# bcsefercik/markerless-robot-camera-calibration

Hardware: AMD Instinct MI355X
Metric: point-cloud frames/sec at 200k pts/frame (higher is better)
Workload: dtype f32

## Files before the change

### markerless-robot-camera-calibration_amd/csrc/sv_conv.hip

```cpp
#include <stdio.h>
#include <stdlib.h>
#include <array>
#include <utility>
#include <vector>

#include "sv_conv_params.h"

namespace sv {

static thread_local char g_last_instance[128] = "";
static thread_local double g_want_scale_override = -1.0;
static thread_local double g_tail_override = -1.0;

constexpr int lds_row_stride(int kc) {
  for (int sa = kc + 2;; ++sa)
    if (sa % 64 == 34 || (sa % 4 == 0 && (sa / 4) % 2 == 1)) return sa;
}

template <int TM_, int WAVES_N, int NT, int CPO = 0>
struct ConvCfg {
  static constexpr ConvTile T = conv_tile(TM_, WAVES_N, NT, CPO);
  static constexpr int WAVES_M = 4 / WAVES_N;
  static constexpr int MR = T.mr, TN = T.tn, GK = T.gk, KC = T.kc, PFD = T.pfd;
  static constexpr bool USE_FULL = T.use_full;
  static constexpr int SA = lds_row_stride(KC);
  static constexpr int F4_PER_ROW = KC / 4;
  static constexpr int ROWS_PER_PASS = 256 / F4_PER_ROW;
  static constexpr int A_F4 = (TM_ + ROWS_PER_PASS - 1) / ROWS_PER_PASS;
  static_assert(MR >= 1, "tile too small for the wave layout");
  static constexpr size_t lds_bytes(int K) { return (size_t)(2 * TM_ * SA + K * TM_) * sizeof(float); }
};

template <int TM_, int WAVES_N, int NT, bool FAST, int CPO = 0, bool RING = false, bool FULL = false>
__device__ __forceinline__ void conv_tile_body(const ConvParams& p, const int bidx, const int tile_base) {
  static_assert(FAST || !FULL, "FULL is a refinement of the FAST form");
  using Cfg = ConvCfg<TM_, WAVES_N, NT, CPO>;
  constexpr int MR = Cfg::MR, TN = Cfg::TN, A_F4 = Cfg::A_F4, KC = Cfg::KC, SA = Cfg::SA, GK = Cfg::GK;
  constexpr int PFD = RING ? Cfg::PFD : 1;
  constexpr int ROWS_PER_PASS = Cfg::ROWS_PER_PASS;
  constexpr int SUBS = TM_ / 16;
  constexpr bool WIDE = FAST && !FULL && !RING && CPO == 0 && WAVES_N == 4 && NT == 3 && (TM_ == 64 || TM_ == 32);
  static_assert(!WIDE || A_F4 == 2, "the WIDE step moves a step's gathers in two halves");
  extern __shared__ __attribute__((aligned(16))) float lds[];
  float* As = lds;
  int* idx_s = (int*)(lds + 2 * TM_ * SA);

  const int tid = threadIdx.x;
  const int lane = tid & 63;
  const int wid = __builtin_amdgcn_readfirstlane(tid >> 6);
  const int wm = wid / WAVES_N, wn = wid % WAVES_N;
  unsigned long long trace_t0 = 0, trace_t_loop = 0, trace_t_epi = 0;
  int trace_steps = 0;
  if (p.trace) trace_t0 = wall_clock64();
  const int ny = (p.Cout + TN - 1) / TN;
  constexpr int SUB_PER_PLAN_TILE = PLAN_TILE / TM_;
  const int t_lin = bidx / ny;
  const int t128 = tile_base + t_lin / SUB_PER_PLAN_TILE;
  const int p128 = p.tile_order ? p.tile_order[t128] : ((int)(p.Vpad / PLAN_TILE) - 1 - t128);
  const int tile = p128 * SUB_PER_PLAN_TILE + (t_lin % SUB_PER_PLAN_TILE);
  const int n0 = (bidx % ny) * TN;
  const int64_t row0 = (int64_t)tile * TM_;
  const int li = lane & 15, lq = lane >> 4;
  const int K = p.K, Cin = p.Cin, Cout = p.Cout;
  const int col0 = n0 + wn * NT * 16 + NT * li;
  const bool cols_full = col0 + NT <= Cout;

  f32x4 acc[MR][NT];
#pragma unroll
  for (int s = 0; s < MR; ++s)
#pragma unroll
    for (int n = 0; n < NT; ++n) acc[s][n] = (f32x4){0.f, 0.f, 0.f, 0.f};

  if (p.acc_init) {
    if constexpr (FAST) {
      const __amdgpu_buffer_rsrc_t rsrc_acc = __builtin_amdgcn_make_buffer_rsrc((void*)p.acc_init, 0, (int)p.acc_bytes, 0x00020000);
      int o_acc[MR][4];
      load_perm_rows<MR>(p, row0 + wm * MR * 16, lane >> 4, o_acc);
#pragma unroll
      for (int s = 0; s < MR; ++s)
#pragma unroll
        for (int reg = 0; reg < 4; ++reg) {
          const auto v = buffer_load_floats<NT>(
              rsrc_acc, o_acc[s][reg] >= 0 ? (uint32_t)o_acc[s][reg] * (uint32_t)(p.acc_ld * 4) + (uint32_t)col0 * 4u : BUF_ABSENT, 0u);
#pragma unroll
          for (int n = 0; n < NT; ++n) acc[s][n][reg] = v[n];
        }
    } else {
#pragma unroll
      for (int s = 0; s < MR; ++s)
#pragma unroll
        for (int reg = 0; reg < 4; ++reg) {
          const int64_t r = row0 + wm * MR * 16 + s * 16 + (lane >> 4) * 4 + reg;
          const int64_t o = p.perm ? (int64_t)p.perm[r] : (r < p.V_out ? r : -1);
#pragma unroll
          for (int n = 0; n < NT; ++n) acc[s][n][reg] = (o >= 0 && col0 + n < Cout) ? p.acc_init[o * p.acc_ld + col0 + n] : 0.0f;
        }
    }
  }
  uint32_t dense_mask = (1u << SUBS) - 1u;
  if (p.submask == nullptr) {
    const int64_t rem = p.V_out - row0;
    const int nsub = rem >= TM_ ? SUBS : (int)((rem + 15) / 16);
    dense_mask = (1u << nsub) - 1u;
  }
  if constexpr (FAST) {
    constexpr int STAGE_IT = (32 * TM_ + 255) / 256;
    int n_st[STAGE_IT];
#pragma unroll
    for (int it = 0; it < STAGE_IT; ++it) {
      const int e = tid + 256 * it;
      const int k = e / TM_, r = e % TM_;
      n_st[it] = -1;
      if (e < K * TM_) {
        if (p.nbr_s)
          n_st[it] = p.nbr_s[(int64_t)k * p.Vpad + row0 + r];
        else
          n_st[it] = (row0 + r < p.V_out) ? (int)(row0 + r) : -1;
      }
    }
#pragma unroll
    for (int it = 0; it < STAGE_IT; ++it) {
      const int e = tid + 256 * it;
      if (e < K * TM_) idx_s[e] = (int)(n_st[it] >= 0 ? (uint32_t)n_st[it] * (uint32_t)(p.in_ld * 4) : BUF_ABSENT);
    }
  } else {
    for (int e = tid; e < K * TM_; e += 256) {
      const int k = e / TM_, r = e - k * TM_;
      int n;
      if (p.nbr_s)
        n = p.nbr_s[(int64_t)k * p.Vpad + row0 + r];
      else
        n = (row0 + r < p.V_out) ? (int)(row0 + r) : -1;
      idx_s[e] = n;
    }
  }
  const __amdgpu_buffer_rsrc_t rsrc_in = __builtin_amdgcn_make_buffer_rsrc((void*)p.in, 0, (int)p.in_bytes, 0x00020000);
  const __amdgpu_buffer_rsrc_t rsrc_w = __builtin_amdgcn_make_buffer_rsrc((void*)p.W, 0, (int)p.w_bytes, 0x00020000);

  const int64_t sm_word = row0 / PLAN_TILE;
  const int sm_shift = (int)((row0 % PLAN_TILE) / 16);
  uint32_t my_sm = 0;
  if (lane < K) my_sm = p.submask ? ((p.submask[sm_word * K + lane] >> sm_shift) & ((1u << SUBS) - 1u)) : dense_mask;
  const uint32_t amask = (uint32_t)__ballot(my_sm != 0);
  auto fused_mask = [&](int k0) -> uint32_t {
    uint32_t m = 0;
#pragma unroll
    for (int g = 0; g < GK; ++g) m |= (uint32_t)__builtin_amdgcn_readlane((int)my_sm, min(k0 + g, 31));
    return m;
  };
  int k_n, c_n = 0;
  uint32_t sm_n = 0;
  bool have_n;
  if (CPO) {
    k_n = 0;
    while (k_n < K && (sm_n = fused_mask(k_n)) == 0) k_n += GK;
    have_n = k_n < K;
  } else {
    k_n = amask ? __builtin_ctz(amask) : K;
    sm_n = amask ? (uint32_t)__builtin_amdgcn_readlane((int)my_sm, k_n) : 0u;
    have_n = amask != 0;
  }
  auto advance = [&]() {
    if (CPO) {
      k_n += GK;
      while (k_n < K && (sm_n = fused_mask(k_n)) == 0) k_n += GK;
      have_n = k_n < K;
      return;
    }
    c_n += KC;
    if (c_n >= Cin) {
      c_n = 0;
      const uint32_t rest = amask & ~((2u << k_n) - 1u);
      have_n = rest != 0;
      k_n = have_n ? __builtin_ctz(rest) : K;
      sm_n = (uint32_t)__builtin_amdgcn_readlane((int)my_sm, have_n ? k_n : 0);
    }
  };

  float4 ra[A_F4];
  const int a_cc = (tid % Cfg::F4_PER_ROW) * 4;
  const int a_r = tid / Cfg::F4_PER_ROW;

  const uint32_t col_bytes = (uint32_t)a_cc * 4u;
  const int cin_rem = Cin % KC;
  const uint32_t col_last = (cin_rem == 0 || a_cc < cin_rem) ? col_bytes : 0u - (uint32_t)(Cin - cin_rem) * 4u;
  auto gather_row = [&](int k, int c0, uint32_t sm, int j) -> float4 {
    const int r = a_r + ROWS_PER_PASS * j;
    if (FAST) {
      const int rr = (A_F4 * ROWS_PER_PASS > TM_) ? min(r, TM_ - 1) : r;
      if (CPO) {
        const int kk = k + a_cc / (CPO ? CPO : 1);
        uint32_t off = (uint32_t)idx_s[min(kk, K - 1) * TM_ + rr];
        if (kk >= K) off = BUF_ABSENT;
        const f32x4 v = buffer_load_floats<4>(rsrc_in, off + (uint32_t)(a_cc % (CPO ? CPO : 1)) * 4u, 0u);
        return make_float4(v[0], v[1], v[2], v[3]);
      } else {
        const uint32_t off = (uint32_t)idx_s[k * TM_ + rr];
        const uint32_t cb = (!FULL && c0 + KC > Cin) ? col_last : col_bytes;
        const f32x4 v = buffer_load_floats<4>(rsrc_in, off + cb, (uint32_t)c0 * 4u);
        return make_float4(v[0], v[1], v[2], v[3]);
      }
      (void)sm;
    } else if (CPO) {
      float e[4] = {0.f, 0.f, 0.f, 0.f};
      if (r < TM_ && ((sm >> (r >> 4)) & 1u)) {
#pragma unroll
        for (int q = 0; q < 4; ++q) {
          const int i = a_cc + q, kk = k + i / (CPO ? CPO : 1), c = i % (CPO ? CPO : 1);
          if (i < GK * CPO && kk < K) {
            const int n = idx_s[kk * TM_ + r];
            if (n >= 0) e[q] = p.in[(int64_t)n * p.in_ld + c];
          }
        }
      }
      return make_float4(e[0], e[1], e[2], e[3]);
    } else {
      float4 v = make_float4(0.f, 0.f, 0.f, 0.f);
      if (r < TM_ && ((sm >> (r >> 4)) & 1u)) {
        const int n = idx_s[k * TM_ + r];
        const int c = c0 + a_cc;
        if (n >= 0) {
          const float* src = p.in + (int64_t)n * p.in_ld + c;
          if (p.vec_a) {
            if (c < Cin) v = *(const float4*)src;
          } else {
            if (c + 0 < Cin) v.x = src[0];
            if (c + 1 < Cin) v.y = src[1];
            if (c + 2 < Cin) v.z = src[2];
            if (c + 3 < Cin) v.w = src[3];
          }
        }
      }
      return v;
    }
  };
  auto load_a = [&](int k, int c0, uint32_t sm) {
#pragma unroll
    for (int j = 0; j < A_F4; ++j) ra[j] = gather_row(k, c0, sm, j);
  };
  auto scatter_row = [&](float* dstbuf, uint32_t sm, int j, const float4& v) {
    const int r = a_r + ROWS_PER_PASS * j;
    if (r < TM_ && (FAST || ((sm >> (r >> 4)) & 1u))) {
      float2* dst = (float2*)(dstbuf + r * SA + a_cc);
      dst[0] = make_float2(v.x, v.y);
      dst[1] = make_float2(v.z, v.w);
    }
  };
  auto store_a = [&](float* dstbuf, uint32_t sm) {
#pragma unroll
    for (int j = 0; j < A_F4; ++j) scatter_row(dstbuf, sm, j, ra[j]);
  };

  typedef float bvec_t __attribute__((ext_vector_type(NT)));
  typedef float bvec_load_t __attribute__((ext_vector_type(NT), aligned(4)));
  constexpr int KS = KC / 4;
  constexpr int BR = WIDE ? 4 : KS;
  bvec_t b[BR];
  const int b_off = lq * Cout + col0;
  const uint32_t b_off_bytes = (uint32_t)b_off * 4u;
  auto step_weights = [&](int k, int c0) -> const float* { return p.W + ((int64_t)k * Cin + c0) * Cout; };
  auto cols_of = [&](int k, int c0) { return CPO ? min(GK, K - k) * CPO : min(KC, Cin - c0); };
  auto ksteps_of = [&](int k, int c0) { return (cols_of(k, c0) + 3) >> 2; };
  auto load_b = [&](const float* wstep, int k, int c0, int ksteps_valid, int ks, bvec_t& dst) {
    if (FAST) {
      const uint32_t row = (uint32_t)(k * Cin + c0 + (ks < ksteps_valid ? 4 * ks : 0));
      dst = buffer_load_floats<NT>(rsrc_w, b_off_bytes, row * (uint32_t)Cout * 4u);
      (void)wstep;
    } else {
      const int i = 4 * ks + lq;
      const float* src = p.W + ((int64_t)k * Cin + c0 + i) * Cout + col0;
      const bool row_ok = i < cols_of(k, c0);
#pragma unroll
      for (int n = 0; n < NT; ++n) dst[n] = (row_ok && col0 + n < Cout) ? src[n] : 0.0f;
    }
  };

  __syncthreads();
  if (have_n) {
    int k_c = k_n, c_c = c_n;
    uint32_t sm_c = sm_n;
    load_a(k_c, c_c, sm_c);
#pragma unroll
    for (int ks = 0; ks < BR; ++ks) load_b(step_weights(k_c, c_c), k_c, c_c, ksteps_of(k_c, c_c), ks, b[ks]);
    store_a(As, sm_c);
    advance();
    int k_x = k_n, c_x = c_n;
    uint32_t sm_x = sm_n;
    bool have_x = have_n;
    __syncthreads();
    int buf = 0;
    if (p.trace) trace_t_loop = wall_clock64();

    auto step = [&]() -> bool {
      if (FAST || have_x) load_a(have_x ? k_x : 0, have_x ? c_x : 0, have_x ? sm_x : 0u);
      const float* a_base = As + buf * (TM_ * SA) + (wm * MR * 16 + li) * SA + lq;
      const uint32_t smw = (sm_c >> (wm * MR)) & ((1u << MR) - 1u);
      const int ksteps = ksteps_of(k_c, c_c);
      const int kb = have_x ? k_x : 0;
      const int cb = have_x ? c_x : 0;
      const float* wnext = step_weights(kb, cb);
      const int ksteps_next = ksteps_of(kb, cb);
      {
        auto reload_b = [&](int ks) {
          if (FULL) {
            b[ks] = buffer_load_floats<NT>(rsrc_w, b_off_bytes, (uint32_t)(kb * Cin + cb + 4 * ks) * (uint32_t)Cout * 4u);
          } else if (FAST || have_x) {
            load_b(wnext, kb, cb, ksteps_next, ks, b[ks]);
          }
        };
        auto mfma_row = [&](int ks, const float (&a)[MR]) {
#pragma unroll
          for (int s = 0; s < MR; ++s) {
            if ((MR == 1 && Cfg::WAVES_M == 1) || ((smw >> s) & 1u)) {
#pragma unroll
              for (int n = 0; n < NT; ++n)
                acc[s][n] = __builtin_amdgcn_mfma_f32_16x16x4f32(a[s], b[ks][n], acc[s][n], 0, 0, 0);
            }
          }
        };
        if constexpr (PFD == 1) {
          float a_cur[MR];
#pragma unroll
          for (int s = 0; s < MR; ++s) a_cur[s] = a_base[s * 16 * SA];
#pragma unroll
          for (int ks = 0; ks < KC / 4; ++ks) {
            if (FULL || ks < ksteps) {
              float a_nx[MR];
              if (ks + 1 < KC / 4) {
#pragma unroll
                for (int s = 0; s < MR; ++s) a_nx[s] = a_base[s * 16 * SA + (ks + 1) * 4];
                if (FULL) __builtin_amdgcn_sched_barrier(0);
              }
              mfma_row(ks, a_cur);
              if (ks + 1 < KC / 4) {
#pragma unroll
                for (int s = 0; s < MR; ++s) a_cur[s] = a_nx[s];
              }
            }
            reload_b(ks);
            if (FULL) __builtin_amdgcn_sched_barrier(0);
          }
        } else {
          float a_ring[PFD + 1][MR];
#pragma unroll
          for (int d = 0; d < PFD; ++d)
#pragma unroll
            for (int s = 0; s < MR; ++s) a_ring[d][s] = a_base[s * 16 * SA + d * 4];
#pragma unroll
          for (int ks = 0; ks < KC / 4; ++ks) {
            if (FULL || ks < ksteps) {
              if (ks + PFD < KC / 4) {
#pragma unroll
                for (int s = 0; s < MR; ++s)
                  a_ring[(ks + PFD) % (PFD + 1)][s] = a_base[s * 16 * SA + (ks + PFD) * 4];
                if (FULL) __builtin_amdgcn_sched_barrier(0);
              }
              mfma_row(ks, a_ring[ks % (PFD + 1)]);
            }
            reload_b(ks);
            if (FULL) __builtin_amdgcn_sched_barrier(0);
          }
        }
      }
      ++trace_steps;
      if (!have_x) return false;
      store_a(As + (buf ^ 1) * (TM_ * SA), sm_x);
      k_c = k_x;
      c_c = c_x;
      sm_c = sm_x;
      advance();
      k_x = k_n;
      c_x = c_n;
      sm_x = sm_n;
      have_x = have_n;
      __syncthreads();
      buf ^= 1;
      return true;
    };
    auto step_wide = [&]() -> bool {
      const int kb = have_x ? k_x : 0;
      const int cb = have_x ? c_x : 0;
      float* const a_next = As + (buf ^ 1) * (TM_ * SA);
      ra[0] = gather_row(kb, cb, 0u, 0);
      const float* a_base = As + buf * (TM_ * SA) + (wm * MR * 16 + li) * SA + lq;
      const uint32_t smw = (sm_c >> (wm * MR)) & ((1u << MR) - 1u);
      const int ksteps = ksteps_of(k_c, c_c);
      const int ksteps_next = ksteps_of(kb, cb);
      const uint32_t wrow_c = (uint32_t)(k_c * Cin + c_c);
      const uint32_t wrow_x = (uint32_t)(kb * Cin + cb);
      float a_cur[MR];
#pragma unroll
      for (int s = 0; s < MR; ++s) a_cur[s] = a_base[s * 16 * SA];
#pragma unroll
      for (int ks = 0; ks < KS; ++ks) {
        if (ks < ksteps) {
          float a_nx[MR];
          if (ks + 1 < KS) {
#pragma unroll
            for (int s = 0; s < MR; ++s) a_nx[s] = a_base[s * 16 * SA + (ks + 1) * 4];
          }
#pragma unroll
          for (int s = 0; s < MR; ++s) {
            if ((smw >> s) & 1u) {
#pragma unroll
              for (int n = 0; n < NT; ++n)
                acc[s][n] = __builtin_amdgcn_mfma_f32_16x16x4f32(a_cur[s], b[ks % BR][n], acc[s][n], 0, 0, 0);
            }
          }
          if (ks + 1 < KS) {
#pragma unroll
            for (int s = 0; s < MR; ++s) a_cur[s] = a_nx[s];
          }
        }
        const int kn = ks + BR < KS ? ks + BR : ks + BR - KS;
        const uint32_t wrow = ks + BR < KS ? wrow_c + (uint32_t)(kn < ksteps ? 4 * kn : 0)
                                           : wrow_x + (uint32_t)(kn < ksteps_next ? 4 * kn : 0);
        b[ks % BR] = buffer_load_floats<NT>(rsrc_w, b_off_bytes, wrow * (uint32_t)Cout * 4u);
        if (ks == KS / 2 - 1) {
          scatter_row(a_next, 0u, 0, ra[0]);
          ra[0] = gather_row(kb, cb, 0u, 1);
        }
      }
      ++trace_steps;
      if (!have_x) return false;
      scatter_row(a_next, 0u, 1, ra[0]);
      k_c = k_x;
      c_c = c_x;
      sm_c = sm_x;
      advance();
      k_x = k_n;
      c_x = c_n;
      sm_x = sm_n;
      have_x = have_n;
      __syncthreads();
      buf ^= 1;
      return true;
    };
    if constexpr (WIDE) {
      while (step_wide()) {
      }
    } else {
      while (step()) {
      }
    }
  }

  if (p.trace) trace_t_epi = wall_clock64();
  float sc[NT], sh[NT];
#pragma unroll
  for (int n = 0; n < NT; ++n) {
    const bool ok = col0 + n < Cout;
    sc[n] = (p.scale && ok) ? p.scale[col0 + n] : 1.0f;
    sh[n] = (p.shift && ok) ? p.shift[col0 + n] : 0.0f;
  }
  if constexpr (FAST) {
    epilogue_buffered<MR, NT>(p, acc, row0 + wm * MR * 16, lq, col0);
  } else
#pragma unroll
  for (int s = 0; s < MR; ++s) {
#pragma unroll
    for (int reg = 0; reg < 4; ++reg) {
      const int64_t r = row0 + wm * MR * 16 + s * 16 + lq * 4 + reg;
      int64_t o;
      if (p.perm)
        o = p.perm[r];
      else
        o = (r < p.V_out) ? r : -1;
      if (o < 0) continue;
      float y[NT];
#pragma unroll
      for (int n = 0; n < NT; ++n) {
        float v = acc[s][n][reg];
        if (p.scale)
          v = __builtin_fmaf(v, sc[n], sh[n]);
        else if (p.shift)
          v = v + sh[n];
        y[n] = v;
      }
      if (p.residual) {
        const float* res = p.residual + o * p.res_ld + col0;
#pragma unroll
        for (int n = 0; n < NT; ++n)
          if (col0 + n < Cout) y[n] = y[n] + res[n];
      }
      float* dst = p.out + o * p.out_ld + col0;
#pragma unroll
      for (int n = 0; n < NT; ++n) {
        float v = y[n];
        if (p.act == SV_ACT_RELU)
          v = v < 0.f ? 0.f : v;
        else if (p.act == SV_ACT_LEAKY_RELU)
          v = v > 0.f ? v : v * p.slope;
        if (col0 + n < Cout) dst[n] = v;
      }
    }
  }
  if (p.trace && tid == 0) {
    unsigned long long* t = p.trace + (size_t)blockIdx.x * 4;
    t[0] = trace_t0;
    t[1] = wall_clock64();
    t[2] = ((unsigned long long)__builtin_amdgcn_s_getreg((31 << 11) | 20) << 32) |
           (unsigned)__builtin_amdgcn_s_getreg((31 << 11) | 4);
    const unsigned long long pro = trace_t_loop ? ((trace_t_loop - trace_t0) >> 4) & 0xffffull : 0ull;
    const unsigned long long epi = ((t[1] - trace_t_epi) >> 4) & 0xffffull;
    t[3] = (unsigned long long)(unsigned)trace_steps | (pro << 32) | (epi << 48);
  }
}

constexpr unsigned wide_waves(int tm, int waves_n, int nt, bool fast, int cpo, bool ring, bool full) {
  return (tm == 64 && waves_n == 4 && nt == 3 && fast && cpo == 0 && !ring && !full) ? 5u : 1u;
}

template <int TM_, int WAVES_N, int NT, bool FAST, int CPO = 0, bool RING = false, bool FULL = false>
__global__ __launch_bounds__(256) __attribute__((amdgpu_waves_per_eu(wide_waves(TM_, WAVES_N, NT, FAST, CPO, RING, FULL))))
void conv_fwd_kernel(ConvParams p) {
  conv_tile_body<TM_, WAVES_N, NT, FAST, CPO, RING, FULL>(p, (int)blockIdx.x, 0);
}

template <int TM_, int TAIL_TM, int WAVES_N, int NT, bool FAST>
__global__ __launch_bounds__(256) __attribute__((amdgpu_waves_per_eu(wide_waves(TM_, WAVES_N, NT, FAST, 0, false, false))))
void conv_fwd_dual_kernel(ConvParams p) {
  if ((int)blockIdx.x < p.main_blocks)
    conv_tile_body<TM_, WAVES_N, NT, FAST>(p, (int)blockIdx.x, 0);
  else
    conv_tile_body<TAIL_TM, WAVES_N, NT, FAST>(p, (int)blockIdx.x - p.main_blocks, p.main_tiles128);
}

template <class Launch>
static int launch_traced(ConvParams& q, unsigned grid, int tm, int wn, int nt, hipStream_t stream, Launch&& launch) {
  static const char* trace_path = getenv("SV_CONV_TRACE");
  q.trace = nullptr;
  if (trace_path) SV_HIP(hipMalloc((void**)&q.trace, (size_t)grid * 4 * sizeof(unsigned long long)));
  launch();
  SV_LAUNCH_CHECK();
  if (q.trace) {
    std::vector<unsigned long long> host((size_t)grid * 4);
    SV_HIP(hipStreamSynchronize(stream));
    SV_HIP(hipMemcpy(host.data(), q.trace, host.size() * sizeof(unsigned long long), hipMemcpyDeviceToHost));
    SV_HIP(hipFree(q.trace));
    if (FILE* f = fopen(trace_path, "ab")) {
      const long long hdr[8] = {0x5356545243ll, (long long)grid, tm, wn, nt, q.ny, q.K, q.Cin};
      fwrite(hdr, sizeof(hdr), 1, f);
      fwrite(host.data(), sizeof(unsigned long long), host.size(), f);
      fclose(f);
    }
  }
  return SV_OK;
}

template <int TM_, int WAVES_N, int NT, int CPO>
static int launch_conv(const ConvParams& p, hipStream_t stream, const ConvChoice& c) {
  using Cfg = ConvCfg<TM_, WAVES_N, NT, CPO>;
  ConvParams q = p;
  q.ntiles = (int)(p.Vpad / TM_);
  q.ny = (p.Cout + Cfg::TN - 1) / Cfg::TN;
  dim3 grid((unsigned)(q.ntiles * q.ny));
  constexpr bool F = (CPO % 4 == 0);
  const size_t lds = Cfg::lds_bytes(p.K);
  return launch_traced(q, grid.x, TM_, WAVES_N, NT, stream, [&] {
    if (c.full) {
      if (c.ring)
        hipLaunchKernelGGL((conv_fwd_kernel<TM_, WAVES_N, NT, F, CPO, (Cfg::PFD > 1), (F && Cfg::USE_FULL)>), grid, dim3(256), lds, stream, q);
      else
        hipLaunchKernelGGL((conv_fwd_kernel<TM_, WAVES_N, NT, F, CPO, false, (F && Cfg::USE_FULL)>), grid, dim3(256), lds, stream, q);
    } else if (c.fast) {
      if (c.ring)
        hipLaunchKernelGGL((conv_fwd_kernel<TM_, WAVES_N, NT, F, CPO, (Cfg::PFD > 1)>), grid, dim3(256), lds, stream, q);
      else
        hipLaunchKernelGGL((conv_fwd_kernel<TM_, WAVES_N, NT, F, CPO, false>), grid, dim3(256), lds, stream, q);
    } else {
      if (c.ring)
        hipLaunchKernelGGL((conv_fwd_kernel<TM_, WAVES_N, NT, false, CPO, (Cfg::PFD > 1)>), grid, dim3(256), lds, stream, q);
      else
        hipLaunchKernelGGL((conv_fwd_kernel<TM_, WAVES_N, NT, false, CPO, false>), grid, dim3(256), lds, stream, q);
    }
  });
}

template <int TM_, int TAIL_TM, int WAVES_N, int NT>
static int launch_conv_dual(const ConvParams& p, hipStream_t stream, const ConvChoice& c) {
  using Main = ConvCfg<TM_, WAVES_N, NT, 0>;
  using Tail = ConvCfg<TAIL_TM, WAVES_N, NT, 0>;
  ConvParams q = p;
  q.ny = p.Cout / Main::TN;
  q.main_tiles128 = (int)(p.Vpad / PLAN_TILE) - c.tail128;
  q.main_blocks = q.main_tiles128 * (PLAN_TILE / TM_) * q.ny;
  q.ntiles = (int)(p.Vpad / TM_);
  const unsigned grid = (unsigned)(q.main_blocks + c.tail128 * (PLAN_TILE / TAIL_TM) * q.ny);
  const size_t lds = Main::lds_bytes(p.K) > Tail::lds_bytes(p.K) ? Main::lds_bytes(p.K) : Tail::lds_bytes(p.K);
  return launch_traced(q, grid, TM_, WAVES_N, NT, stream, [&] {
    hipLaunchKernelGGL((conv_fwd_dual_kernel<TM_, TAIL_TM, WAVES_N, NT, true>), dim3(grid), dim3(256), lds, stream, q);
  });
}

typedef int (*ConvLauncher)(const ConvParams&, hipStream_t, const ConvChoice&);
template <size_t... I>
static constexpr std::array<ConvLauncher, sizeof...(I)> conv_launchers(std::index_sequence<I...>) {
  return {{&launch_conv<CONV_TILES[I].tm, CONV_TILES[I].wn, CONV_TILES[I].nt, CONV_TILES[I].cpo>...}};
}
static constexpr auto CONV_LAUNCHERS = conv_launchers(std::make_index_sequence<N_CONV_TILES>{});

static bool forced_tile(const ConvShape& s, int& tile) {
  int tm = 0, wn = 0, nt = 0, cpo = 0, cout = 0;
  long long vmin = 0, vmax = 0;
  const char* f;
  bool hit = false;
  if ((f = getenv("SV_CONV_FORCE_RANGE")))
    hit = sscanf(f, "%lld:%lld:%d:%d,%d,%d", &vmin, &vmax, &cout, &tm, &wn, &nt) == 6 && s.Vpad >= vmin && s.Vpad <= vmax &&
          s.Cout == cout && s.K > 1;
  if (!hit && (f = getenv("SV_CONV_FORCE_DENSE")))
    hit = sscanf(f, "%lld:%d:%d,%d,%d", &vmin, &cout, &tm, &wn, &nt) == 5 && s.Vpad >= vmin && s.Cout == cout && s.K == 1;
  if (!hit && (f = getenv("SV_CONV_FORCE")))
    hit = sscanf(f, "%d,%d,%d,%d", &tm, &wn, &nt, &cpo) >= 3;
  if (!hit) return false;
  tile = find_conv_tile(tm, wn, nt, cpo);
  if (tile < 0) set_error("sv_conv_fwd: no kernel instance <%d,%d,%d> cpo %d", tm, wn, nt, cpo);
  return true;
}

static void effective_dispatch(double& want_scale, double& tail_fraction) {
  static const double env_want_scale =
      getenv("SV_CONV_WANT_SCALE") ? atof(getenv("SV_CONV_WANT_SCALE")) : SV_CONV_WANT_SCALE_DEFAULT;
  static const double env_tail = getenv("SV_CONV_TAIL") ? atof(getenv("SV_CONV_TAIL")) : SV_CONV_TAIL_DEFAULT;
  want_scale = g_want_scale_override >= 0.0 ? g_want_scale_override : env_want_scale;
  tail_fraction = g_tail_override >= 0.0 ? g_tail_override : env_tail;
}

static int launch_choice(const ConvChoice& c, const ConvParams& p, hipStream_t stream) {
  switch (c.kind) {
    case CONV_FIRST_MFMA: return launch_conv_first_mfma(p, stream);
    case CONV_FIRST_LAYER: return launch_conv_first_layer(p, stream);
    case CONV_THIN: return launch_conv_thin(p, stream);
    case CONV_THIN_LDS: return launch_conv_thin_lds(p, stream);
    case CONV_NARROW: return launch_linear_narrow(p, stream);
    case CONV_DUAL: return launch_conv_dual<64, 32, 4, 3>(p, stream, c);
    default: return CONV_LAUNCHERS[find_conv_tile(c.tm, c.wn, c.nt, c.cpo)](p, stream, c);
  }
}

}

using namespace sv;

extern "C" const char* sv_conv_last_instance(void) { return sv::g_last_instance; }

extern "C" int sv_conv_set_dispatch(double want_scale, double tail_fraction) {
  SV_CHECK_ARG(tail_fraction < 1.0, "tail_fraction must be below 1");
  sv::g_want_scale_override = want_scale;
  sv::g_tail_override = tail_fraction;
  return SV_OK;
}

extern "C" int sv_conv_fwd(const float* in, int64_t V_in, int64_t in_ld, int Cin, const float* W, int K, int Cout,
                           const int32_t* perm, const int32_t* nbr_s, const uint32_t* submask,
                           const int32_t* tile_order, int64_t V_out, int64_t Vpad, const float* scale, const float* shift, const float* residual, int64_t res_ld,
                           int act, float slope, float* out, int64_t out_ld, sv_stream_t stream_) {
  return sv_conv_fwd_acc(in, V_in, in_ld, Cin, W, K, Cout, perm, nbr_s, submask, tile_order, V_out, Vpad, nullptr, 0, scale, shift,
                         residual, res_ld, act, slope, out, out_ld, stream_);
}

extern "C" int sv_conv_fwd_acc(const float* in, int64_t V_in, int64_t in_ld, int Cin, const float* W, int K, int Cout,
                               const int32_t* perm, const int32_t* nbr_s, const uint32_t* submask, const int32_t* tile_order,
                               int64_t V_out, int64_t Vpad, const float* acc_init, int64_t acc_ld, const float* scale,
                               const float* shift, const float* residual, int64_t res_ld, int act, float slope, float* out,
                               int64_t out_ld, sv_stream_t stream_) {
  hipStream_t stream = (hipStream_t)stream_;
  SV_CHECK_ARG(!acc_init || acc_ld >= Cout, "acc_init stride too small");
  SV_CHECK_ARG(Cin > 0 && Cout > 0 && K >= 1 && K <= 32, "bad channel / kernel volume");
  SV_CHECK_ARG(V_out >= 0 && Vpad >= V_out && Vpad % PLAN_TILE == 0, "Vpad must be a multiple of 128 >= V_out");
  SV_CHECK_ARG(in_ld >= Cin && out_ld >= Cout, "row strides too small");
  SV_CHECK_ARG(act >= SV_ACT_NONE && act <= SV_ACT_LEAKY_RELU, "bad activation");
  if (V_out == 0) return SV_OK;
  SV_CHECK_ARG(in && W && out, "null pointer");
  SV_CHECK_ARG(V_in >= 1, "V_in = rows of `in` (every index of the plan is below it)");
  const bool has_plan = perm || nbr_s || submask;
  SV_CHECK_ARG(!has_plan || (perm && nbr_s && submask), "perm, nbr_s and submask must be given together");
  SV_CHECK_ARG(has_plan || K == 1, "K > 1 needs a plan");
  SV_CHECK_ARG(!residual || res_ld >= Cout, "residual stride too small");
  ConvParams p;
  p.in = in; p.in_ld = in_ld; p.Cin = Cin; p.W = W; p.K = K; p.Cout = Cout;
  p.perm = perm; p.nbr_s = nbr_s; p.submask = submask; p.tile_order = tile_order; p.V_out = V_out; p.Vpad = Vpad;
  p.scale = scale; p.shift = shift; p.residual = residual; p.res_ld = res_ld;
  p.acc_init = acc_init; p.acc_ld = acc_ld;
  p.act = act; p.slope = slope; p.out = out; p.out_ld = out_ld;
  p.vec_a = (in_ld % 4 == 0) && (Cin % 4 == 0) && (((uintptr_t)in & 15) == 0);
  const uint64_t in_bytes = ((uint64_t)(V_in - 1) * (uint64_t)in_ld + (uint64_t)Cin) * 4u;
  const uint64_t w_bytes = (uint64_t)K * (uint64_t)Cin * (uint64_t)Cout * 4u;
  const uint64_t out_bytes = ((uint64_t)(V_out - 1) * (uint64_t)out_ld + (uint64_t)Cout) * 4u;
  const uint64_t res_bytes = residual ? ((uint64_t)(V_out - 1) * (uint64_t)res_ld + (uint64_t)Cout) * 4u : 0u;
  const uint64_t acc_bytes = acc_init ? ((uint64_t)(V_out - 1) * (uint64_t)acc_ld + (uint64_t)Cout) * 4u : 0u;
  p.buf_ok = in_bytes < BUF_LIMIT && w_bytes < BUF_LIMIT && out_bytes < BUF_LIMIT && res_bytes < BUF_LIMIT &&
             acc_bytes < BUF_LIMIT && (((uintptr_t)perm & 15) == 0);
  p.acc_bytes = p.buf_ok ? (uint32_t)acc_bytes : 0u;
  if (!p.buf_ok && !has_plan && K == 1 && w_bytes < BUF_LIMIT) {
    int64_t ld_max = in_ld > out_ld ? in_ld : out_ld;
    if (residual && res_ld > ld_max) ld_max = res_ld;
    const int64_t rows = (int64_t)((BUF_LIMIT - 4096u) / ((uint64_t)ld_max * 4u)) / PLAN_TILE * PLAN_TILE;
    if (rows >= PLAN_TILE && rows < V_out) {
      for (int64_t r0 = 0; r0 < V_out; r0 += rows) {
        const int64_t n = V_out - r0 < rows ? V_out - r0 : rows;
        const int rc = sv_conv_fwd_acc(in + r0 * in_ld, n, in_ld, Cin, W, K, Cout, nullptr, nullptr, nullptr, nullptr, n,
                                       (n + PLAN_TILE - 1) / PLAN_TILE * PLAN_TILE, acc_init ? acc_init + r0 * acc_ld : nullptr,
                                       acc_ld, scale, shift, residual ? residual + r0 * res_ld : nullptr, res_ld, act, slope,
                                       out + r0 * out_ld, out_ld, stream_);
        if (rc != SV_OK) return rc;
      }
      return SV_OK;
    }
  }
  p.in_bytes = p.buf_ok ? (uint32_t)in_bytes : 0u;
  p.w_bytes = p.buf_ok ? (uint32_t)w_bytes : 0u;
  p.out_bytes = p.buf_ok ? (uint32_t)out_bytes : 0u;
  p.res_bytes = p.buf_ok ? (uint32_t)res_bytes : 0u;
  p.ntiles = 0;
  p.ny = 0;
  p.trace = nullptr;
  p.main_blocks = 0;
  p.main_tiles128 = 0;
  const ConvShape shape = {K, Cin, Cout, Vpad, has_plan, tile_order != nullptr, p.vec_a != 0, p.buf_ok != 0, acc_init != nullptr,
                           ((uintptr_t)W & 15) == 0, g_want_scale_override >= 1.0};
  double want_scale, tail_fraction;
  effective_dispatch(want_scale, tail_fraction);
  ConvChoice c = conv_select(shape, want_scale, tail_fraction);
  int forced;
  if ((c.kind == CONV_TILE || c.kind == CONV_DUAL) && forced_tile(shape, forced)) {
    if (forced < 0) return SV_ERR_INVALID;
    c = conv_tile_form(CONV_TILES[forced], shape);
  }
  const int rc = launch_choice(c, p, stream);
  if (rc == SV_OK) conv_choice_name(c, g_last_instance, sizeof(g_last_instance));
  return rc;
}

extern "C" int sv_conv_select(int64_t n, const int64_t* shapes_host, double want_scale, double tail_fraction, char* names_host,
                              size_t name_bytes) {
  SV_CHECK_ARG(n >= 0 && (n == 0 || (shapes_host && names_host)) && name_bytes > 0, "null pointer");
  SV_CHECK_ARG(tail_fraction < 1.0, "tail_fraction must be below 1");
  double ws, tf;
  effective_dispatch(ws, tf);
  const bool alone = want_scale >= 0.0 ? want_scale >= 1.0 : g_want_scale_override >= 1.0;
  if (want_scale >= 0.0) ws = want_scale;
  if (tail_fraction >= 0.0) tf = tail_fraction;
  for (int64_t i = 0; i < n; ++i) {
    const int64_t* s = shapes_host + 5 * i;
    const int64_t K = s[0], Cin = s[1], Cout = s[2], Vpad = s[3], flags = s[4];
    SV_CHECK_ARG(Cin > 0 && Cin <= INT32_MAX && Cout > 0 && Cout <= INT32_MAX && K >= 1 && K <= 32, "bad channel / kernel volume");
    SV_CHECK_ARG(Vpad > 0 && Vpad % PLAN_TILE == 0, "Vpad must be a positive multiple of 128");
    SV_CHECK_ARG((flags & SV_CONV_SEL_PLAN) || K == 1, "K > 1 needs a plan");
    SV_CHECK_ARG(!(flags & SV_CONV_SEL_VEC_A) || Cin % 4 == 0, "float4 gathers need Cin % 4 == 0");
    const ConvShape shape = {(int)K, (int)Cin, (int)Cout, Vpad, (flags & SV_CONV_SEL_PLAN) != 0, (flags & SV_CONV_SEL_TILE_ORDER) != 0,
                             (flags & SV_CONV_SEL_VEC_A) != 0, (flags & SV_CONV_SEL_BUF_OK) != 0, (flags & SV_CONV_SEL_ACC_INIT) != 0,
                             (flags & SV_CONV_SEL_W_ALIGNED) != 0, alone};
    conv_choice_name(conv_select(shape, ws, tf), names_host + (size_t)i * name_bytes, name_bytes);
  }
  return SV_OK;
}

extern "C" int sv_conv_tile_info(int index, int* out_host) {
  SV_CHECK_ARG(index >= 0 && index < N_CONV_TILES, "no such row of the tile table");
  SV_CHECK_ARG(out_host, "null pointer");
  const ConvTile& t = CONV_TILES[index];
  const int row[10] = {t.tm, t.wn, t.nt, t.cpo, t.mr, t.tn, t.gk, t.kc, t.pfd, (int)t.use_full};
  for (int i = 0; i < 10; ++i) out_host[i] = row[i];
  return SV_OK;
}
```

Measured before the change: 74.74.

## Interleave k-step pairs in LDS A tile for float2 reads in wide step

Adds a dedicated LDS row layout for the WIDE conv step. Values for consecutive k-steps are interleaved in pairs with an XOR swizzle, so each lane reads two k-steps of A with one 8-byte ds_read instead of two 4-byte reads. The scatter path writes the matching swizzled layout and the MFMA loop now walks k-step pairs. The aim is to halve the LDS read instructions and avoid bank conflicts, at the cost of more complex scatter addressing and a possibly different row stride.

```diff
diff --git a/markerless-robot-camera-calibration_amd/csrc/sv_conv.hip b/markerless-robot-camera-calibration_amd/csrc/sv_conv.hip
--- a/markerless-robot-camera-calibration_amd/csrc/sv_conv.hip
+++ b/markerless-robot-camera-calibration_amd/csrc/sv_conv.hip
@@ -15,6 +15,14 @@
 constexpr int lds_row_stride(int kc) {
   for (int sa = kc + 2;; ++sa)
     if (sa % 64 == 34 || (sa % 4 == 0 && (sa / 4) % 2 == 1)) return sa;
+}
+
+constexpr int lds_row_stride_wide(int kc) {
+  for (int sa = kc;; ++sa)
+    if (sa % 4 == 0 && (sa / 4) % 2 == 1) return sa;
+}
+constexpr int wide_a_word(int r, int ks, int lq, int saw) {
+  return r * saw + 8 * (ks / 2) + 2 * (lq ^ (((r >> 1) ^ (ks >> 3)) & 1)) + ks % 2;
 }
 
 template <int TM_, int WAVES_N, int NT, int CPO = 0>
@@ -24,23 +32,28 @@
   static constexpr int MR = T.mr, TN = T.tn, GK = T.gk, KC = T.kc, PFD = T.pfd;
   static constexpr bool USE_FULL = T.use_full;
   static constexpr int SA = lds_row_stride(KC);
+  static constexpr bool HAS_WIDE = CPO == 0 && WAVES_N == 4 && NT == 3 && (TM_ == 64 || TM_ == 32);
+  static constexpr int SAW = HAS_WIDE ? lds_row_stride_wide(KC) : SA;
   static constexpr int F4_PER_ROW = KC / 4;
   static constexpr int ROWS_PER_PASS = 256 / F4_PER_ROW;
   static constexpr int A_F4 = (TM_ + ROWS_PER_PASS - 1) / ROWS_PER_PASS;
   static_assert(MR >= 1, "tile too small for the wave layout");
-  static constexpr size_t lds_bytes(int K) { return (size_t)(2 * TM_ * SA + K * TM_) * sizeof(float); }
+  static constexpr size_t lds_bytes(int K) { return (size_t)(2 * TM_ * (SA > SAW ? SA : SAW) + K * TM_) * sizeof(float); }
 };
 
 template <int TM_, int WAVES_N, int NT, bool FAST, int CPO = 0, bool RING = false, bool FULL = false>
 __device__ __forceinline__ void conv_tile_body(const ConvParams& p, const int bidx, const int tile_base) {
   static_assert(FAST || !FULL, "FULL is a refinement of the FAST form");
   using Cfg = ConvCfg<TM_, WAVES_N, NT, CPO>;
-  constexpr int MR = Cfg::MR, TN = Cfg::TN, A_F4 = Cfg::A_F4, KC = Cfg::KC, SA = Cfg::SA, GK = Cfg::GK;
+  constexpr int MR = Cfg::MR, TN = Cfg::TN, A_F4 = Cfg::A_F4, KC = Cfg::KC, GK = Cfg::GK;
   constexpr int PFD = RING ? Cfg::PFD : 1;
   constexpr int ROWS_PER_PASS = Cfg::ROWS_PER_PASS;
   constexpr int SUBS = TM_ / 16;
   constexpr bool WIDE = FAST && !FULL && !RING && CPO == 0 && WAVES_N == 4 && NT == 3 && (TM_ == 64 || TM_ == 32);
   static_assert(!WIDE || A_F4 == 2, "the WIDE step moves a step's gathers in two halves");
+  static_assert(!WIDE || (Cfg::HAS_WIDE && A_F4 * ROWS_PER_PASS == TM_ && KC % 16 == 0 && KC <= 64),
+                "the WIDE row layout: whole passes of rows, k-step pairs, one swizzle bit for pairs 4..7");
+  constexpr int SA = WIDE ? Cfg::SAW : Cfg::SA;
   extern __shared__ __attribute__((aligned(16))) float lds[];
   float* As = lds;
   int* idx_s = (int*)(lds + 2 * TM_ * SA);
@@ -238,8 +251,22 @@
 #pragma unroll
     for (int j = 0; j < A_F4; ++j) ra[j] = gather_row(k, c0, sm, j);
   };
+  const int a_ks = tid % Cfg::F4_PER_ROW;
+  const int wide_w0 = a_r * SA + 8 * (a_ks >> 1) + (a_ks & 1) + 2 * (((a_r >> 1) ^ (a_ks >> 3)) & 1);
+  const int wide_w1 = wide_w0 ^ 2;
+  static_assert(!WIDE || (ROWS_PER_PASS % 4 == 0 && SA % 4 == 0), "one swizzle bit per thread, 8-byte aligned pairs");
   auto scatter_row = [&](float* dstbuf, uint32_t sm, int j, const float4& v) {
     const int r = a_r + ROWS_PER_PASS * j;
+    if constexpr (WIDE) {
+      float* d0 = dstbuf + ROWS_PER_PASS * j * SA + wide_w0;
+      float* d1 = dstbuf + ROWS_PER_PASS * j * SA + wide_w1;
+      d0[0] = v.x;
+      d0[4] = v.z;
+      d1[0] = v.y;
+      d1[4] = v.w;
+      (void)sm;
+      return;
+    }
     if (r < TM_ && (FAST || ((sm >> (r >> 4)) & 1u))) {
       float2* dst = (float2*)(dstbuf + r * SA + a_cc);
       dst[0] = make_float2(v.x, v.y);
@@ -378,45 +405,58 @@
       return true;
     };
     auto step_wide = [&]() -> bool {
+      constexpr int NP = KS / 2;
       const int kb = have_x ? k_x : 0;
       const int cb = have_x ? c_x : 0;
       float* const a_next = As + (buf ^ 1) * (TM_ * SA);
       ra[0] = gather_row(kb, cb, 0u, 0);
-      const float* a_base = As + buf * (TM_ * SA) + (wm * MR * 16 + li) * SA + lq;
+      const int a_sw = (li >> 1) & 1;
+      const float* a_base[2];
+      a_base[0] = As + buf * (TM_ * SA) + (wm * MR * 16 + li) * SA + 2 * (lq ^ a_sw);
+      a_base[1] = As + buf * (TM_ * SA) + (wm * MR * 16 + li) * SA + 2 * (lq ^ a_sw ^ 1);
+      auto a_read = [&](int q) -> float2 {
+        return *(const float2*)(a_base[((q / MR) >> 2) & 1] + (q % MR) * 16 * SA + 8 * (q / MR));
+      };
       const uint32_t smw = (sm_c >> (wm * MR)) & ((1u << MR) - 1u);
       const int ksteps = ksteps_of(k_c, c_c);
       const int ksteps_next = ksteps_of(kb, cb);
       const uint32_t wrow_c = (uint32_t)(k_c * Cin + c_c);
       const uint32_t wrow_x = (uint32_t)(kb * Cin + cb);
-      float a_cur[MR];
-#pragma unroll
-      for (int s = 0; s < MR; ++s) a_cur[s] = a_base[s * 16 * SA];
-#pragma unroll
-      for (int ks = 0; ks < KS; ++ks) {
-        if (ks < ksteps) {
-          float a_nx[MR];
-          if (ks + 1 < KS) {
-#pragma unroll
-            for (int s = 0; s < MR; ++s) a_nx[s] = a_base[s * 16 * SA + (ks + 1) * 4];
-          }
-#pragma unroll
-          for (int s = 0; s < MR; ++s) {
-            if ((smw >> s) & 1u) {
-#pragma unroll
-              for (int n = 0; n < NT; ++n)
-                acc[s][n] = __builtin_amdgcn_mfma_f32_16x16x4f32(a_cur[s], b[ks % BR][n], acc[s][n], 0, 0, 0);
-            }
-          }
-          if (ks + 1 < KS) {
-#pragma unroll
-            for (int s = 0; s < MR; ++s) a_cur[s] = a_nx[s];
-          }
-        }
+      float2 a[MR];
+#pragma unroll
+      for (int s = 0; s < MR; ++s) a[s] = a_read(s);
+      auto reload_b = [&](int ks) {
         const int kn = ks + BR < KS ? ks + BR : ks + BR - KS;
         const uint32_t wrow = ks + BR < KS ? wrow_c + (uint32_t)(kn < ksteps ? 4 * kn : 0)
                                            : wrow_x + (uint32_t)(kn < ksteps_next ? 4 * kn : 0);
         b[ks % BR] = buffer_load_floats<NT>(rsrc_w, b_off_bytes, wrow * (uint32_t)Cout * 4u);
-        if (ks == KS / 2 - 1) {
+      };
+#pragma unroll
+      for (int p = 0; p < NP; ++p) {
+        if (2 * p < ksteps) {
+#pragma unroll
+          for (int s = 0; s < MR; ++s) {
+            if ((smw >> s) & 1u) {
+#pragma unroll
+              for (int n = 0; n < NT; ++n)
+                acc[s][n] = __builtin_amdgcn_mfma_f32_16x16x4f32(a[s].x, b[(2 * p) % BR][n], acc[s][n], 0, 0, 0);
+            }
+          }
+        }
+        reload_b(2 * p);
+        if (2 * p + 1 < ksteps) {
+#pragma unroll
+          for (int s = 0; s < MR; ++s) {
+            if ((smw >> s) & 1u) {
+#pragma unroll
+              for (int n = 0; n < NT; ++n)
+                acc[s][n] = __builtin_amdgcn_mfma_f32_16x16x4f32(a[s].y, b[(2 * p + 1) % BR][n], acc[s][n], 0, 0, 0);
+            }
+            if (p + 1 < NP) a[s] = a_read((p + 1) * MR + s);
+          }
+        }
+        reload_b(2 * p + 1);
+        if (p == NP / 2 - 1) {
           scatter_row(a_next, 0u, 0, ra[0]);
           ra[0] = gather_row(kb, cb, 0u, 1);
         }
```

New measurement: 75.46 (median of 6 runs). Within noise of the previous version (+1.0%).
